# GewelsJI/MVLT

Measured on AMD Instinct MI355X. Metric: image-text pairs/sec/node, PVT-tiny MVLT pre-train step, higher is better.
Workload: dtype bf16

## Files before the change

mvlt_amd/_lib.py:

```python
import ctypes as C
import os

import torch

_HERE = os.path.dirname(os.path.abspath(__file__))
LIB_PATH = os.environ.get("MVLT_HIP_LIB") or os.path.join(_HERE, "libmvlt_hip.so")


class MVLTError(RuntimeError):
    pass


if not os.path.exists(LIB_PATH):
    raise ImportError(f"{LIB_PATH} is missing: build it with `python -m mvlt_amd.build` (hipcc, gfx950). "
                      "mvlt_amd has no CPU or eager fallback.")
lib = C.CDLL(LIB_PATH)

c_int, c_float, c_void_p, c_long = C.c_int, C.c_float, C.c_void_p, C.c_long


class RowMap(C.Structure):
    _fields_ = [(n, c_int) for n in ("mode", "rows_per_batch", "batch_stride", "offset",
                                     "r", "w_in", "tokens_in", "hw_out", "w_out", "c_seg", "h_in")]

# ... 140 lines not shown
    "mvlt_upsample_fwd": (_i, [_vp, _i, _i, _i, _i, _i, _i, _vp, _i, _i, _i, _vp]),
    "mvlt_upsample_bwd": (_i, [_vp, _i, _i, _i, _i, _i, _i, _i, _vp, _i, _i, _i, _i, _vp]),
    "mvlt_upsample_l1_fwd": (_i, [_vp, _i, _i, _i, _i, _i, _i, _vp, _vp, _vp]),
    "mvlt_upsample_l1_bwd": (_i, [_vp, _i, _i, _i, _i, _i, _i, _vp, _vp, _vp, _i, _i, _vp]),
}
EXPORTS = list(PROTOTYPES)
for _name, (_res, _args) in PROTOTYPES.items():
    _fn = getattr(lib, _name)
    _fn.restype, _fn.argtypes = _res, _args

ABI_VERSION = 8
if lib.mvlt_abi_version() != ABI_VERSION:
    raise ImportError(f"ABI mismatch: {LIB_PATH} is version {lib.mvlt_abi_version()}, the binding is version {ABI_VERSION} (stale build? run python -m mvlt_amd.build)")
for _name, _cls in STRUCTS:
    _n = lib.mvlt_sizeof(_name.encode())
    if _n != C.sizeof(_cls):
        raise ImportError(f"ABI mismatch for {_name}: library says {_n} bytes, binding has {C.sizeof(_cls)}")

EXT_PROTOTYPES = {
    "mvlt_ext_version": (_i, []),
    "mvlt_step_gate": (_i, [_vp, _i, _f, _f, _vp, _vp, _vp]),
    "mvlt_adamw_step_gated": (_i, [_vp, _vp, _vp, _vp, _vp, _l, _vp, _vp, _vp, _vp]),
}
for _name, (_res, _args) in EXT_PROTOTYPES.items():
    if not hasattr(lib, _name):
        raise ImportError(f"{LIB_PATH} does not export {_name} (include/mvlt_hip_ext.h): stale build? run python -m mvlt_amd.build")
    _fn = getattr(lib, _name)
    _fn.restype, _fn.argtypes = _res, _args

EXT_VERSION = 1
if lib.mvlt_ext_version() != EXT_VERSION:
    raise ImportError(f"extension mismatch: {LIB_PATH} is version {lib.mvlt_ext_version()}, the binding is version {EXT_VERSION} (stale build? run python -m mvlt_amd.build)")

DT = {torch.bfloat16: 0, torch.float32: 1}


def last_kernel():
    s = lib.mvlt_last_kernel().decode()
    s = s.replace("(anonymous namespace)::", "")
    if s.startswith("void "):
        s = s[5:]
    depth = 0
    for i, ch in enumerate(s):
        depth += ch == "<"
        depth -= ch == ">"
        if ch == "(" and depth == 0:
            return s[:i]
    return s


def check(rc, what):
    if rc != 0:
        raise MVLTError(f"{what} failed ({rc}): {lib.mvlt_last_error().decode()}")


_raw_stream, _cur_device = torch._C._cuda_getCurrentRawStream, torch._C._cuda_getDevice


def stream_ptr():
    return _raw_stream(_cur_device())


def ptr(t):
    if t is None:
        return None
    if not t.is_cuda:
# ... 15 lines not shown
```

mvlt_amd/build.py:

```python
import concurrent.futures
import os
import subprocess
import sys

HERE = os.path.dirname(os.path.abspath(__file__))
CSRC = os.path.join(HERE, "csrc")
OBJ = os.path.join(HERE, "csrc", "_obj")
LIB = os.path.join(HERE, "libmvlt_hip.so")
ARCH = "gfx950"
FLAGS = ["--offload-arch=" + ARCH, "-O3", "-std=c++17", "-fPIC", "-ffp-contract=fast", "-Wno-unused-result"]
EXTRA = {"mlp.hip": ["-fno-slp-vectorize"]}


def _sources():
    return sorted(f for f in os.listdir(CSRC) if f.endswith(".hip"))


def source_hash():
    import hashlib
    h = hashlib.sha256()
    files = sorted(os.path.join(CSRC, f) for f in os.listdir(CSRC) if f.endswith((".hip", ".h", ".inc")))
    files += [os.path.join(HERE, "..", "include", h) for h in ("mvlt_hip.h", "mvlt_hip_ext.h")]
    for f in files:
        h.update(os.path.basename(f).encode())
        h.update(open(f, "rb").read())
    return h.hexdigest()[:16]


def _deps_mtime():
    hdrs = [os.path.join(CSRC, f) for f in os.listdir(CSRC) if f.endswith((".h", ".inc"))]
    hdrs += [os.path.join(HERE, "..", "include", h) for h in ("mvlt_hip.h", "mvlt_hip_ext.h")]
    return max(os.path.getmtime(h) for h in hdrs)


def _compile(src, force, verbose):
    s = os.path.join(CSRC, src)
    o = os.path.join(OBJ, src[:-4] + ".o")
    if not force and os.path.exists(o) and os.path.getmtime(o) >= max(os.path.getmtime(s), _deps_mtime()):
        return o
    cmd = ["hipcc", *FLAGS, *EXTRA.get(src, []), "-c", s, "-o", o]
    if verbose:
        print(" ".join(cmd), flush=True)
    r = subprocess.run(cmd, capture_output=True, text=True)
    if r.returncode != 0:
        raise RuntimeError(f"hipcc failed for {src}:\n{r.stdout}\n{r.stderr}")
    return o


def build(force=False, verbose=False):
    os.makedirs(OBJ, exist_ok=True)
    srcs = _sources()
    with concurrent.futures.ThreadPoolExecutor(max_workers=min(6, len(srcs))) as ex:
        objs = list(ex.map(lambda s: _compile(s, force, verbose), srcs))
    if force or not os.path.exists(LIB) or any(os.path.getmtime(o) > os.path.getmtime(LIB) for o in objs):
        cmd = ["hipcc", "--offload-arch=" + ARCH, "-shared", "-fPIC", *objs, "-o", LIB]
        if verbose:
            print(" ".join(cmd), flush=True)
        r = subprocess.run(cmd, capture_output=True, text=True)
        if r.returncode != 0:
            raise RuntimeError(f"link failed:\n{r.stdout}\n{r.stderr}")
    return LIB


if __name__ == "__main__":
# ... 2 lines not shown
```

mvlt_amd/csrc/elementwise.hip:

```cpp
#include "common.h"
#include "../../include/mvlt_hip.h"
#include "../../include/mvlt_hip_ext.h"

namespace {

constexpr int NT = 256;

template <typename T, int HID>
__global__ __launch_bounds__(NT) void bert_embed_fwd_kernel(const long* ids, const float* word, const float* pos, const float* type0,
                                                            const float* gamma, const float* beta, const uint8_t* keep, float inv_keep,
                                                            T* y, float* mean_out, float* rstd_out, int rows, int Tlen, float eps) {
  constexpr int PER = HID / 64;
  const int lane = threadIdx.x & 63;
  const int row = blockIdx.x * (NT / 64) + (threadIdx.x >> 6);
  if (row >= rows) return;
  const long id = ids[row];
  const int t = row % Tlen;
  float v[PER];
  float s = 0.f;
#pragma unroll
  for (int i = 0; i < PER; ++i) {
    int c = lane + 64 * i;
    v[i] = word[id * HID + c] + type0[c] + pos[(long)t * HID + c];
    s += v[i];
  }
  const float mean = wave_sum(s) * (1.0f / HID);
  float q = 0.f;
#pragma unroll
  for (int i = 0; i < PER; ++i) { float d = v[i] - mean; q += d * d; }
  const float rstd = rsqrtf(wave_sum(q) * (1.0f / HID) + eps);
  if (lane == 0) { mean_out[row] = mean; rstd_out[row] = rstd; }
#pragma unroll
  for (int i = 0; i < PER; ++i) {
    int c = lane + 64 * i;
    float o = (v[i] - mean) * rstd * gamma[c] + beta[c];
// ... 261 lines not shown
    loss_sum[0] += L;
    count[0] += Cn;
  }
}

template <typename T, typename TO>
__global__ __launch_bounds__(NT) void ce_bwd_kernel(const T* logits, const long* labels, long ignore, const float* lse, const float* gscale,
                                                    const float* count, TO* dlogits, int rows, int V, int ld, int ldd) {
  const int row = blockIdx.x;
  const T* lr = logits + (long)row * ld;
  TO* dr = dlogits + (long)row * ldd;
  const long lab = labels[row];
  const float l = lse[row];
  const float sc = (lab == ignore) ? 0.f : gscale[0] / fmaxf(count[0], 1.0f);
  int c_first = 0;
  if constexpr (sizeof(T) == 4) {
    if ((ld & 3) == 0 && (ldd & 3) == 0 && (((uintptr_t)logits) & 15) == 0 && (((uintptr_t)dlogits) & 15) == 0) {
      const int V4 = V & ~3;
      for (int c = threadIdx.x * 4; c < V4; c += NT * 4) {
        const f32x4 x = *(const f32x4*)((const float*)lr + c);
        f32x4 g;
#pragma unroll
        for (int e = 0; e < 4; ++e) g[e] = (__expf(x[e] - l) - (c + e == lab ? 1.f : 0.f)) * sc;
        if constexpr (sizeof(TO) == 2) *(bf16x4*)((bf16*)dr + c) = bf16x4{(bf16)g[0], (bf16)g[1], (bf16)g[2], (bf16)g[3]};
        else *(f32x4*)((float*)dr + c) = g;
      }
      c_first = V4;
    }
  }
  for (int c = c_first + threadIdx.x; c < ldd; c += NT) {
    float g = 0.f;
    if (c < V) g = (__expf((float)lr[c] - l) - (c == lab ? 1.f : 0.f)) * sc;
    dr[c] = (TO)g;
  }
}

__global__ __launch_bounds__(NT) void smooth_l1_sum_kernel(const float* pred, const float* target, long n, float* loss_sum) {
  __shared__ float s_w[NT / 64];
  float acc = 0.f;
  const long stride = (long)gridDim.x * NT * 4;
  long i = ((long)blockIdx.x * NT + threadIdx.x) * 4;
  for (; i + 3 * stride < n; i += 4 * stride) {
    f32x4 a[4], b[4];
#pragma unroll
    for (int u = 0; u < 4; ++u) { a[u] = *(const f32x4*)(pred + i + u * stride); b[u] = *(const f32x4*)(target + i + u * stride); }
#pragma unroll
    for (int u = 0; u < 4; ++u)
#pragma unroll
      for (int e = 0; e < 4; ++e) {
        const float d = fabsf(a[u][e] - b[u][e]);
        acc += d < 1.0f ? 0.5f * d * d : d - 0.5f;
      }
  }
  for (; i < n; i += stride) {
    const f32x4 a = *(const f32x4*)(pred + i), b = *(const f32x4*)(target + i);
#pragma unroll
    for (int e = 0; e < 4; ++e) {
      const float d = fabsf(a[e] - b[e]);
      acc += d < 1.0f ? 0.5f * d * d : d - 0.5f;
    }
  }
  acc = wave_sum(acc);
  if ((threadIdx.x & 63) == 0) s_w[threadIdx.x >> 6] = acc;
  __syncthreads();
  if (threadIdx.x == 0) {
    float t = 0.f;
// ... 552 lines not shown

extern "C" int mvlt_smooth_l1_fwd(const float* pred, const float* target, long n, float* loss_sum, void* stream) {
  MVLT_REQUIRE(pred && target && loss_sum && n > 0 && n % 4 == 0 && (((uintptr_t)pred | (uintptr_t)target) & 15) == 0,
               "mvlt_smooth_l1_fwd: bad arguments (n multiple of 4, 16-byte aligned)");
  MVLT_LAUNCH(smooth_l1_sum_kernel, dim3(grid_for(n / 4, 2048)), dim3(NT), 0, (hipStream_t)stream, pred, target, n, loss_sum);
  return mvlt_check_launch("mvlt_smooth_l1_fwd");
}

extern "C" int mvlt_smooth_l1_bwd(const float* pred, const float* target, long n, const float* gscale, float* grad, void* stream) {
  MVLT_REQUIRE(pred && target && gscale && grad && n > 0 && n % 4 == 0 && (((uintptr_t)pred | (uintptr_t)target | (uintptr_t)grad) & 15) == 0,
               "mvlt_smooth_l1_bwd: bad arguments (n multiple of 4, 16-byte aligned)");
  MVLT_LAUNCH(smooth_l1_grad_kernel, dim3(grid_for(n / 4, 8192)), dim3(NT), 0, (hipStream_t)stream, pred, target, n, gscale, 1.0f / (float)n, grad);
  return mvlt_check_launch("mvlt_smooth_l1_bwd");
}

extern "C" int mvlt_adamw_step(float* p, const float* g, float* m, float* v, void* p_bf16, long n, const float* hp,
                               const uint8_t* decay_mask, const float* gscale_dev, void* stream) {
  MVLT_REQUIRE(p && g && m && v && hp && n >= 0 && n % 4 == 0, "mvlt_adamw_step: bad arguments (n must be a multiple of 4)");
  if (n == 0) return MVLT_OK;
  MVLT_LAUNCH((adamw_kernel<false>), dim3(grid_for(n / 4, 8192)), dim3(NT), 0, (hipStream_t)stream, p, g, m, v, (bf16*)p_bf16, n, hp, decay_mask, gscale_dev);
  return mvlt_check_launch("mvlt_adamw_step");
}

extern "C" int mvlt_ext_version(void) { return MVLT_EXT_VERSION; }

extern "C" int mvlt_adamw_step_gated(float* p, const float* g, float* m, float* v, void* p_bf16, long n, const float* hp,
                                     const uint8_t* decay_mask, const float* gate, void* stream) {
  MVLT_REQUIRE(p && g && m && v && hp && gate && n >= 0 && n % 4 == 0, "mvlt_adamw_step_gated: bad arguments (null pointer, or n is not a multiple of 4)");
  if (n == 0) return MVLT_OK;
  MVLT_LAUNCH((adamw_kernel<true>), dim3(grid_for(n / 4, 8192)), dim3(NT), 0, (hipStream_t)stream, p, g, m, v, (bf16*)p_bf16, n, hp, decay_mask, gate);
  return mvlt_check_launch("mvlt_adamw_step_gated");
}

extern "C" int mvlt_step_gate(const float* partials, int n_partials, float grad_scale, float max_norm, float* out, int* counters, void* stream) {
  MVLT_REQUIRE(partials && out && counters, "mvlt_step_gate: null pointer (partials, out and counters are required)");
  MVLT_REQUIRE(n_partials >= 1 && n_partials <= 1024, "mvlt_step_gate: n_partials must be in [1, 1024], got %d", n_partials);
  MVLT_LAUNCH(step_gate_kernel, dim3(1), dim3(NT), 0, (hipStream_t)stream, partials, n_partials, grad_scale, max_norm, out, counters);
  return mvlt_check_launch("mvlt_step_gate");
}

extern "C" int mvlt_grad_sumsq(const float* g, long n, const uint8_t* mask, float* partials, int n_partials, void* stream) {
  MVLT_REQUIRE(g && partials && n >= 0 && n % 4 == 0, "mvlt_grad_sumsq: bad arguments (n must be a multiple of 4)");
  MVLT_REQUIRE(n_partials >= 1 && n_partials <= 1024, "mvlt_grad_sumsq: n_partials must be in [1, 1024], got %d", n_partials);
  MVLT_REQUIRE(((uintptr_t)g & 15) == 0 && ((uintptr_t)mask & 3) == 0, "mvlt_grad_sumsq: g must be 16-byte aligned, mask 4-byte aligned");
  if (mask) MVLT_LAUNCH((grad_sumsq_kernel<true>), dim3(n_partials), dim3(NT), 0, (hipStream_t)stream, g, n, mask, partials);
  else MVLT_LAUNCH((grad_sumsq_kernel<false>), dim3(n_partials), dim3(NT), 0, (hipStream_t)stream, g, n, mask, partials);
  return mvlt_check_launch("mvlt_grad_sumsq");
}

extern "C" int mvlt_clip_coef(const float* partials, int n_partials, float grad_scale, float max_norm, float* out, void* stream) {
  MVLT_REQUIRE(partials && out && n_partials >= 1 && n_partials <= 1024, "mvlt_clip_coef: bad arguments (n_partials must be in [1, 1024])");
  MVLT_LAUNCH(clip_coef_kernel, dim3(1), dim3(NT), 0, (hipStream_t)stream, partials, n_partials, grad_scale, max_norm, out);
  return mvlt_check_launch("mvlt_clip_coef");
}

extern "C" int mvlt_scale_by_dev(float* x, long n, const float* factor_dev, void* stream) {
  MVLT_REQUIRE(x && factor_dev && n >= 0 && n % 4 == 0 && ((uintptr_t)x & 15) == 0, "mvlt_scale_by_dev: bad arguments (n must be a multiple of 4, x 16-byte aligned)");
  if (n == 0) return MVLT_OK;
  MVLT_LAUNCH(scale_by_dev_kernel, dim3(grid_for(n / 4, 8192)), dim3(NT), 0, (hipStream_t)stream, x, n, factor_dev);
  return mvlt_check_launch("mvlt_scale_by_dev");
}

extern "C" int mvlt_cast_bf16(const float* src, void* dst, long n, void* stream) {
  MVLT_REQUIRE(src && dst && n >= 0 && n % 4 == 0, "mvlt_cast_bf16: bad arguments (n must be a multiple of 4)");
  if (n == 0) return MVLT_OK;
  MVLT_LAUNCH(cast_f32_bf16_kernel, dim3(grid_for(n / 4, 8192)), dim3(NT), 0, (hipStream_t)stream, src, (bf16*)dst, n);
// ... 54 lines not shown
```

mvlt_amd/engine.py:

```python
import math

import torch
import torch.nn.functional as F

from ._lib import MVLTError
from .metrics import MetricLogger, SmoothedValue
from .params import pool_zeros

MLM_LOSS_WEIGHT, ITM_LOSS_WEIGHT, T2I_LOSS_WEIGHT = 1, 1, 10
USE_ORI_INPUT_IDS = False


def _core(model):
    return model.module if hasattr(model, "module") else model


class _SmoothL1Fn(torch.autograd.Function):

    @staticmethod
    def forward(ctx, pred, target):
        from . import ops
        pred, target = pred.contiguous(), target.contiguous()
        acc = pool_zeros((1,), torch.float32, pred.device)
        ops.smooth_l1_fwd(pred, target, acc)
# ... 152 lines not shown
        self.pin.copy_(vals, non_blocking=True)
        self.ev.record()

    def get(self):
        self.ev.synchronize()
        return self.pin.tolist()


def to_device_batch(samples, device):
    keys = ("image", "mlm_labels", "i2t_labels", "masked_images", "itm_labels", "sup_cls_labels", "sub_cls_labels")
    batch = {k: samples[k].to(device, non_blocking=True) for k in keys if k in samples}
    batch["input_ids"] = samples["ori_input_ids" if USE_ORI_INPUT_IDS else "input_ids"].to(device, non_blocking=True)
    if "mlm_positions" in samples:
        batch["mlm_positions"] = samples["mlm_positions"].to(device, non_blocking=True)
    if "mlm_count" in samples:
        batch["mlm_count"] = int(samples["mlm_count"])
    elif "mlm_positions" not in samples and not samples["mlm_labels"].is_cuda:
        batch["mlm_count"] = int((samples["mlm_labels"] != -1).sum())
    return batch


def train_one_epoch_vl(model, criterion, data_loader, optimizer, device, epoch, loss_scaler, max_norm=0,
                       model_ema=None, mixup_fn=None, set_training_mode=True, fp32=False, args=None):
    model.train(set_training_mode)
    core = _core(model)
    if fp32 and getattr(core, "compute_dtype", None) not in (None, torch.float32):
        core.set_compute_dtype(torch.float32)
    logger = MetricLogger(delimiter="  ")
    logger.add_meter("lr", SmoothedValue(window_size=1, fmt="{value:.6f}"))
    header = f"Epoch: [{epoch}]"
    loss_type = getattr(args, "loss_type", None) or core.loss_type
    t2i_on = loss_type.get("t2i", 0) == 1
    readback = _LossReadback()
    for idx, samples in enumerate(logger.log_every(data_loader, 10, header)):
        batch = to_device_batch(samples, device)
        total, parts = train_step(model, batch, idx, t2i_on)
        readback.post(total, parts)
        optimizer.zero_grad()
        is_second_order = hasattr(optimizer, "is_second_order") and optimizer.is_second_order
        loss_scaler(total, optimizer, clip_grad=max_norm, parameters=model.parameters(), create_graph=is_second_order)
        if model_ema is not None:
            model_ema.update(model)
        vals = readback.get()
        if not math.isfinite(vals[0]):
            print(f" [ Warning!!! ] Total Loss is {vals[0]} (loss_mlm={vals[1]} | loss_itm={vals[2]} | loss_sup_cls={vals[3]} | "
                  f"loss_sub_cls={vals[4]} | loss_t2i={vals[5]}), non-finite value"
                  + (" -- the step is guarded: non-finite gradients skip the optimizer step" if getattr(loss_scaler, "skip_nonfinite", False) else ""))
        logger.update(**dict(zip(LOSS_KEYS, vals)))
        logger.update(lr=optimizer.param_groups[0]["lr"])
    logger.synchronize_between_processes(device)
    print("Averaged stats:", logger)
    return {k: m.global_avg for k, m in logger.meters.items()}


train_one_epoch = train_one_epoch_vl


class BF16Scaler:
    state_dict_key = "amp_scaler"

    def __init__(self, skip_nonfinite=False):
        self._scaler = None
        self.skip_nonfinite = bool(skip_nonfinite)
        self.skipped_steps = 0
        self.last_grad_norm = None

    def __call__(self, loss, optimizer, clip_grad=None, parameters=None, create_graph=False):
        from .optim import FusedAdamW
        store = optimizer.model.store if isinstance(optimizer, FusedAdamW) else None
        self.last_grad_norm = None
        if store is not None:
            store.scale_in_optimizer = True
        try:
            loss.backward(create_graph=create_graph)
            if self.skip_nonfinite and store is not None:
                self.last_grad_norm = store.gate_grads(clip_grad or None)
            elif self.skip_nonfinite:
                assert parameters is not None
                parameters = list(parameters)
                norm = torch.nn.utils.clip_grad_norm_(parameters, clip_grad if clip_grad else float("inf"))
                if not math.isfinite(float(norm)):
                    self.skipped_steps += 1
                    return
            elif clip_grad and store is not None:
                self.last_grad_norm = store.clip_grad_norm(clip_grad)
            elif clip_grad:
                assert parameters is not None
                parameters = list(parameters)
                torch.nn.utils.clip_grad_norm_(parameters, clip_grad)
            optimizer.step()
        finally:
            if store is not None:
                store.scale_in_optimizer = False
                store.apply_pending_scale()

    def state_dict(self):
        return {}

    def load_state_dict(self, sd):
        pass
```

mvlt_amd/ops.py:

```python
import ctypes as C

import torch

from . import _lib as L
from ._lib import DT, check, patchmap, ptr, rowmap, stream_ptr

_ID = rowmap()


def gemm_nt(A, B, C_out, M, N, K, lda, ldb, ldc, *, a_map=None, c_map=None, bias=None, act=0, H=None,
            row_scale=None, rows_per_scale=0, R=None, col_sum=None, col_sumsq=None, col_copies=0, split_k=0, post_ln=None):
    assert A.dtype == B.dtype and A.dtype in DT and (C_out.dtype in DT or (C_out.dtype == torch.float16 and col_sum is not None))
    if bias is not None:
        assert bias.dtype == torch.float32
    if row_scale is not None:
        assert row_scale.dtype == torch.float32
    if R is not None:
        assert R.dtype == C_out.dtype or (R.dtype == torch.float32 and C_out.dtype == torch.bfloat16)
    if H is not None:
        assert H.dtype == C_out.dtype
    if col_sum is not None:
        assert col_sum.dtype == torch.float32 and col_sumsq is not None and col_sumsq.dtype == torch.float32
    a = L.GemmNTArgs(A=ptr(A), B=ptr(B), C=ptr(C_out), M=M, N=N, K=K, lda=lda, ldb=ldb, ldc=ldc,
                     dtype=DT[A.dtype], out_dtype=2 if C_out.dtype == torch.float16 else DT[C_out.dtype], a_map=a_map or _ID, c_map=c_map or _ID,
# ... 155 lines not shown


def masked_select(labels, idx, count, ignore_index=-1):
    assert labels.dtype == torch.int64 and idx.dtype == torch.int32 and count.dtype == torch.int32 and labels.is_contiguous()
    check(L.lib.mvlt_masked_select(ptr(labels), labels.numel(), ignore_index, ptr(idx), ptr(count), stream_ptr()), "mvlt_masked_select")


def gather_rows(src, idx, dst, rows, Cdim, ld_src, src_map=None):
    assert idx.dtype == torch.int32 and src.dtype == dst.dtype
    m = C.byref(src_map) if src_map is not None else None
    check(L.lib.mvlt_gather_rows(ptr(src), ptr(idx), ptr(dst), rows, Cdim, ld_src, m, DT[src.dtype], stream_ptr()), "mvlt_gather_rows")
    return dst


def scatter_rows(src, idx, dst, rows, Cdim, ld_dst, dst_map=None, accumulate=False):
    assert idx.dtype == torch.int32 and src.dtype == dst.dtype
    m = C.byref(dst_map) if dst_map is not None else None
    check(L.lib.mvlt_scatter_rows(ptr(src), ptr(idx), ptr(dst), rows, Cdim, ld_dst, m, 1 if accumulate else 0, DT[src.dtype], stream_ptr()),
          "mvlt_scatter_rows")
    return dst


def cross_entropy_fwd(logits, labels, lse, loss_sum, count, rows, V, ld, ignore_index=-1):
    assert labels.dtype == torch.int64
    check(L.lib.mvlt_cross_entropy_fwd(ptr(logits), ptr(labels), ignore_index, ptr(lse), ptr(loss_sum), ptr(count), rows, V, ld,
                                       DT[logits.dtype], stream_ptr()), "mvlt_cross_entropy_fwd")


def cross_entropy_bwd(logits, labels, lse, gscale, count, dlogits, rows, V, ld, ldd, ignore_index=-1):
    check(L.lib.mvlt_cross_entropy_bwd(ptr(logits), ptr(labels), ignore_index, ptr(lse), ptr(gscale), ptr(count), ptr(dlogits), rows, V, ld, ldd,
                                       DT[logits.dtype], DT[dlogits.dtype], stream_ptr()), "mvlt_cross_entropy_bwd")


ADAMW_FROZEN = 2


def adamw_step(p, g, m, v, p16, n, hp, decay_mask=None, *, gscale_dev=None):
    assert decay_mask is None or decay_mask.dtype == torch.uint8
    if gscale_dev is not None:
        assert gscale_dev.dtype == torch.float32
    check(L.lib.mvlt_adamw_step(ptr(p), ptr(g), ptr(m), ptr(v), ptr(p16), n, ptr(hp), ptr(decay_mask), ptr(gscale_dev), stream_ptr()), "mvlt_adamw_step")


def grad_sumsq(g, n, mask, partials):
    assert g.dtype == torch.float32 and partials.dtype == torch.float32 and g.is_contiguous() and partials.is_contiguous()
    assert g.numel() >= n and (mask is None or (mask.dtype == torch.uint8 and mask.is_cuda and mask.is_contiguous() and mask.numel() >= n))
    check(L.lib.mvlt_grad_sumsq(ptr(g), n, ptr(mask), ptr(partials), partials.numel(), stream_ptr()), "mvlt_grad_sumsq")


def clip_coef(partials, grad_scale, max_norm, out):
    assert partials.dtype == torch.float32 and out.dtype == torch.float32 and out.numel() >= 2 and out.is_contiguous() and partials.is_contiguous()
    check(L.lib.mvlt_clip_coef(ptr(partials), partials.numel(), float(grad_scale), float(max_norm), ptr(out), stream_ptr()), "mvlt_clip_coef")


def step_gate(partials, grad_scale, max_norm, out, counters):
    assert partials.dtype == torch.float32 and out.dtype == torch.float32 and out.numel() >= 4 and out.is_contiguous() and partials.is_contiguous()
    assert counters.dtype == torch.int32 and counters.numel() >= 2 and counters.is_contiguous()
    check(L.lib.mvlt_step_gate(ptr(partials), partials.numel(), float(grad_scale), float(max_norm), ptr(out), ptr(counters), stream_ptr()), "mvlt_step_gate")


def adamw_step_gated(p, g, m, v, p16, n, hp, decay_mask, gate):
    assert decay_mask is None or decay_mask.dtype == torch.uint8
    assert gate.dtype == torch.float32 and gate.numel() >= 4 and gate.is_contiguous()
    check(L.lib.mvlt_adamw_step_gated(ptr(p), ptr(g), ptr(m), ptr(v), ptr(p16), n, ptr(hp), ptr(decay_mask), ptr(gate), stream_ptr()), "mvlt_adamw_step_gated")


# ... 221 lines not shown
```

mvlt_amd/params.py:

```python
import math
import weakref
from collections import OrderedDict

import torch
import torch.nn as nn

from . import ops

_TN_SCRATCH_MIB = 256
ALIGN = 8


class Holder(nn.Module):

    def __init__(self, **shapes):
        super().__init__()
        for name, shape in shapes.items():
            self.register_parameter(name, nn.Parameter(torch.zeros(*shape)))


def affine(n):
    return Holder(weight=(n,), bias=(n,))


# ... 62 lines not shown
        self.used += nbytes
        return t


def pool_zeros(shape, dtype, device):
    return ZeroPool.of(torch.device(device) if not isinstance(device, torch.device) else device).take(tuple(shape) if not isinstance(shape, int) else (shape,), dtype)


class FlatStore:

    def __init__(self, module, compute_dtype):
        self.module = module
        self.compute_dtype = compute_dtype
        self.device = None
        self.P = self.G = self.C = None
        self._views = {}
        self.offsets = OrderedDict()
        self.params = OrderedDict()
        self.total = 0
        self._cast_version = -1
        self.refresh_count = 0
        self._c_fresh_version = None
        self.extra = {}
        self._finalize_queued = False
        self.force_dirty = True
        self.fn_params = []
        self.on_backward_done = None
        self.on_range_ready = None
        self.on_pass_aborted = None
        self._ranges_done = []
        self.all_zeroed_this_pass = False
        self.touched_this_pass = set()
        self.scale_in_optimizer = False
        self.pending_grad_scale = 1.0
        self.pending_clip = None
        self._clip = None
        self.pending_gate = None
        self._gate = None
        self.grad_works = []

    def _index(self):
        self.offsets.clear()
        self.params.clear()
        off = 0
        seen = set()
        for name, p in self.module.named_parameters():
            if id(p) in seen:
                continue
            seen.add(id(p))
            n = p.numel()
            self.offsets[name] = (off, n, tuple(p.shape))
            self.params[name] = p
            off += (n + ALIGN - 1) // ALIGN * ALIGN
        self.total = off
        self.fn_params = list(self.params.items())

    def is_current(self):
        if self.P is None:
            return False
        for name in (next(iter(self.params)), next(reversed(self.params))):
            off, n, _ = self.offsets[name]
            if self.params[name].data_ptr() != self.P.data_ptr() + 4 * off:
                return False
        return True

    def materialize(self, device):
# ... 377 lines not shown
```

mvlt_amd/schedule.py:

```python
import torch
import torch.nn.functional as F

from . import ops
from ._lib import patchmap, rowmap
from .params import ZeroPool, pool_zeros
from .pvlt import BERT_DROP, EPS_BERT, EPS_BLOCK, EPS_DEFAULT, VOCAB, VOCAB_LD


def _empty(shape, dtype, dev):
    return torch.empty(shape, dtype=dtype, device=dev)


def conv_wgrad(S, name, dz, xin, M, cout, K, ld_dz, ld_in, bmap, taps, cin, colsum=None):
    ops.gemm_tn(dz, xin, S.grad_taps(name, cout, taps, cin), M, cout, K, ld_dz, ld_in, K, b_map=bmap, colsum=colsum, partials=S.tn_partials(), defer_fold=True)


def _step_rng(model):
    model._rng_calls = getattr(model, "_rng_calls", 0) + 1
    return torch.initial_seed(), model._rng_calls


def check_input_size(model, Himg, Wimg):
    unit = model.patch_size * 8
    assert Himg % unit == 0 and Wimg % unit == 0, \
# ... 815 lines not shown
    @staticmethod
    def backward(ctx, dlogits):
        model, HW, x4, e, sv_e, t, sv_t, a_map, sink = ctx.pack
        S, dt, dev = model.store, model.compute_dtype, x4.device
        S.queue_finalize()
        B, N, C = x4.shape
        T = N - HW
        R = B * T
        dl = torch.zeros(R, VOCAB_LD, device=dev, dtype=dt)
        dl[:, :VOCAB] = dlogits.reshape(R, VOCAB).to(dt)
        u = ctx.unit
        dx4, ret = (sink or _GradSink(S)).take(x4.shape, dt, dev) if u.dgrad else (None, None)
        _mlm_decoder_bwd(model, dl, t, sv_t, e, sv_e, x4, a_map, R, C, dx4, accumulate=True, unit=u)
        ctx.pack = ctx.unit = None
        return ret, None, None, None


def _mlm_decoder_bwd(model, dl, t, sv_t, e, sv_e, A, a_map, R, lda, dA, c_map=None, accumulate=False, unit=_EVERY):
    S, dt, dev = model.store, model.compute_dtype, dl.device
    Hd = model.hidden
    wname = WORD_TABLE
    if unit.launches["table"]:
        ops.gemm_tn(dl, t, S.grad(wname), R, VOCAB, Hd, VOCAB_LD, Hd, Hd, colsum=S.grad("mlm_head.bias"),
                    overwrite=dt == torch.bfloat16 and S.all_zeroed_this_pass and wname not in S.touched_this_pass)
        S.touched_this_pass.add(wname)
    elif unit.launches["bias"]:
        db = _empty((1, VOCAB_LD), torch.float32, dev)
        ops.batch_sum(dl, db, R, 1, VOCAB_LD, 1, VOCAB_LD)
        S.grad("mlm_head.bias").add_(db[0, :VOCAB])
    wT = S.extra[wname + "::T"]
    if dt == torch.bfloat16:
        dtr32 = pool_zeros((R, Hd), torch.float32, dev)
        ops.gemm_nt(dl, wT, dtr32, R, Hd, VOCAB_LD, VOCAB_LD, VOCAB_LD, Hd, split_k=4)
        dtr = dtr32.to(dt)
    else:
        dtr = _empty((R, Hd), dt, dev)
        ops.gemm_nt(dl, wT, dtr, R, Hd, VOCAB_LD, VOCAB_LD, VOCAB_LD, Hd)
    de = _mlm_transform_bwd(model, dtr, sv_t, e, R, unit)
    _embed_ln_bwd(model, "mlm_head_embed", de, sv_e, A, a_map, R, lda, dA, c_map if c_map is not None else a_map, accumulate, unit)
    S.announce_prefix("mlm_head_embed.", "mlm_head.")


class _MLMFusedFn(torch.autograd.Function):

    @staticmethod
    def forward(ctx, x4, model, HW, positions, labels_sel, sink):
        S, dt, dev = model.store, model.compute_dtype, x4.device
        B, N, C = x4.shape
        T = N - HW
        R = positions.numel()
        rows = _empty((R, C), dt, dev)
        tmap = rowmap(T, N, HW)
        ops.gather_rows(x4, positions, rows, R, C, C, src_map=tmap)
        e, sv_e = _embed_ln_fwd(model, "mlm_head_embed", rows, None, R, C)
        t, sv_t = _mlm_transform_fwd(model, e, R)
        logits = _empty((R, VOCAB_LD), torch.float32, dev)
        ops.gemm_nt(t, S.comp("text_embeddings.word_embeddings.weight"), logits, R, VOCAB, model.hidden, model.hidden, model.hidden, VOCAB_LD,
                    bias=S.master("mlm_head.bias"))
        lse = _empty((R,), torch.float32, dev)
        acc = pool_zeros((2,), torch.float32, dev)
        ops.cross_entropy_fwd(logits, labels_sel, lse, acc[0:1], acc[1:2], R, VOCAB, VOCAB_LD)
        ctx.pack = (model, HW, x4.shape, rows, e, sv_e, t, sv_t, logits, lse, acc, positions, labels_sel, tmap, sink)
        ctx.unit = _unit(getattr(model, "_plan", None), "mlm_head")
        return acc[0] / acc[1]

    @staticmethod
    def backward(ctx, gloss):
        model, HW, xshape, rows, e, sv_e, t, sv_t, logits, lse, acc, positions, labels_sel, tmap, sink = ctx.pack
        S, dt, dev = model.store, model.compute_dtype, rows.device
        S.queue_finalize()
        B, N, C = xshape
        R = positions.numel()
        dl = _empty((R, VOCAB_LD), dt, dev)
        gs = gloss.reshape(1).float().contiguous()
        ops.cross_entropy_bwd(logits, labels_sel, lse, gs, acc[1:2], dl, R, VOCAB, VOCAB_LD, VOCAB_LD)
        u = ctx.unit
        drows = _empty((R, C), dt, dev) if u.dgrad else None
        _mlm_decoder_bwd(model, dl, t, sv_t, e, sv_e, rows, None, R, C, drows, c_map=None, unit=u)
        ret = None
        if u.dgrad:
            dx4, ret = (sink or _GradSink(S)).take(xshape, dt, dev)
            ops.scatter_rows(drows, positions, dx4, R, C, C, dst_map=tmap, accumulate=True)
        ctx.pack = ctx.unit = None
        return ret, None, None, None, None, None


class _HostCount:
    _pins = {}

    def __init__(self, cnt):
        key = (cnt.device.index, cnt.numel())
        pin = self._pins.get(key)
        if pin is None:
            pin = self._pins[key] = torch.empty(cnt.numel(), dtype=cnt.dtype).pin_memory()
        self.pin = pin
        pin.copy_(cnt, non_blocking=True)
        self.ev = torch.cuda.Event()
        self.ev.record()

    def get(self):
        self.ev.synchronize()
        return int(self.pin[0])


def run_forward(model, images, ids, mlm_labels=None, mlm_positions=None, mlm_count=None, t2i_target=None):
    S = model.store
    dev = images.device
    grad_on = _begin_pass(model, dev)
# ... 77 lines not shown
```

Measured before the change: 13520.

## Fuse MLM cross-entropy forward and backward into one kernel during forward

Adds a fused HIP kernel that computes the log-sum-exp and writes the logit gradient in a single pass over each row, launched in the forward pass with a precomputed upstream loss weight. This saves re-reading the fp32 logits in backward and one kernel launch, and lets the logits buffer be freed early. The backward path only rescales the gradient if the promised upstream weight was not honoured. It also swaps a torch dtype conversion for the library's bf16 cast op. The risk is that gradients are wrong if the actual upstream scale differs from the announced weight, and the extra plumbing across engine, store and schedule makes that easy to get out of sync.

```diff
diff --git a/include/mvlt_hip_ext2.h b/include/mvlt_hip_ext2.h
--- /dev/null
+++ b/include/mvlt_hip_ext2.h
@@ -0,0 +1,19 @@
+#ifndef MVLT_HIP_EXT2_H
+#define MVLT_HIP_EXT2_H
+#include <stdint.h>
+#ifdef __cplusplus
+extern "C" {
+#endif
+
+#define MVLT_EXT2_VERSION 1
+int mvlt_ext2_version(void);
+
+#define MVLT_CE_FUSED_MAX_V 32768
+#define MVLT_CE_FUSED_MAX_GRID 2048
+int mvlt_cross_entropy_fwd_bwd(const void* logits, const long* labels, long ignore_index, float* lse, float* loss_sum, float* count,
+                               const float* gscale , void* dlogits, int rows, int V, int ld, int ldd, int dtype, int out_dtype, void* stream);
+
+#ifdef __cplusplus
+}
+#endif
+#endif
diff --git a/mvlt_amd/_lib.py b/mvlt_amd/_lib.py
--- a/mvlt_amd/_lib.py
+++ b/mvlt_amd/_lib.py
@@ -196,6 +196,20 @@
 if lib.mvlt_ext_version() != EXT_VERSION:
     raise ImportError(f"extension mismatch: {LIB_PATH} is version {lib.mvlt_ext_version()}, the binding is version {EXT_VERSION} (stale build? run python -m mvlt_amd.build)")
 
+EXT2_PROTOTYPES = {
+    "mvlt_ext2_version": (_i, []),
+    "mvlt_cross_entropy_fwd_bwd": (_i, [_vp, _vp, _l, _vp, _vp, _vp, _vp, _vp, _i, _i, _i, _i, _i, _i, _vp]),
+}
+for _name, (_res, _args) in EXT2_PROTOTYPES.items():
+    if not hasattr(lib, _name):
+        raise ImportError(f"{LIB_PATH} does not export {_name} (include/mvlt_hip_ext2.h): stale build? run python -m mvlt_amd.build)")
+    _fn = getattr(lib, _name)
+    _fn.restype, _fn.argtypes = _res, _args
+
+EXT2_VERSION = 1
+if lib.mvlt_ext2_version() != EXT2_VERSION:
+    raise ImportError(f"extension mismatch: {LIB_PATH} is version {lib.mvlt_ext2_version()} of mvlt_hip_ext2.h, the binding is version {EXT2_VERSION} (stale build? run python -m mvlt_amd.build)")
+
 DT = {torch.bfloat16: 0, torch.float32: 1}
 
 
diff --git a/mvlt_amd/build.py b/mvlt_amd/build.py
--- a/mvlt_amd/build.py
+++ b/mvlt_amd/build.py
@@ -10,6 +10,7 @@
 ARCH = "gfx950"
 FLAGS = ["--offload-arch=" + ARCH, "-O3", "-std=c++17", "-fPIC", "-ffp-contract=fast", "-Wno-unused-result"]
 EXTRA = {"mlp.hip": ["-fno-slp-vectorize"]}
+ABI_HEADERS = ("mvlt_hip.h", "mvlt_hip_ext.h", "mvlt_hip_ext2.h")
 
 
 def _sources():
@@ -20,7 +21,7 @@
     import hashlib
     h = hashlib.sha256()
     files = sorted(os.path.join(CSRC, f) for f in os.listdir(CSRC) if f.endswith((".hip", ".h", ".inc")))
-    files += [os.path.join(HERE, "..", "include", h) for h in ("mvlt_hip.h", "mvlt_hip_ext.h")]
+    files += [os.path.join(HERE, "..", "include", h) for h in ABI_HEADERS]
     for f in files:
         h.update(os.path.basename(f).encode())
         h.update(open(f, "rb").read())
@@ -29,7 +30,7 @@
 
 def _deps_mtime():
     hdrs = [os.path.join(CSRC, f) for f in os.listdir(CSRC) if f.endswith((".h", ".inc"))]
-    hdrs += [os.path.join(HERE, "..", "include", h) for h in ("mvlt_hip.h", "mvlt_hip_ext.h")]
+    hdrs += [os.path.join(HERE, "..", "include", h) for h in ABI_HEADERS]
     return max(os.path.getmtime(h) for h in hdrs)
 
 
diff --git a/mvlt_amd/csrc/elementwise.hip b/mvlt_amd/csrc/elementwise.hip
--- a/mvlt_amd/csrc/elementwise.hip
+++ b/mvlt_amd/csrc/elementwise.hip
@@ -1,6 +1,7 @@
 #include "common.h"
 #include "../../include/mvlt_hip.h"
 #include "../../include/mvlt_hip_ext.h"
+#include "../../include/mvlt_hip_ext2.h"
 
 namespace {
 
@@ -328,6 +329,103 @@
     float g = 0.f;
     if (c < V) g = (__expf((float)lr[c] - l) - (c == lab ? 1.f : 0.f)) * sc;
     dr[c] = (TO)g;
+  }
+}
+
+constexpr int CE_NT = 1024;
+template <typename T, typename TO, int NCH>
+__global__ __launch_bounds__(CE_NT) void ce_fwd_bwd_kernel(const T* logits, const long* labels, long ignore, float* lse, const float* gscale,
+                                                           TO* dlogits, int rows, int V, int ld, int ldd) {
+  constexpr int PC = 16 / sizeof(T), NW = CE_NT / 64;
+  __shared__ float s_m[NW], s_s[NW];
+  __shared__ int s_c[NW];
+  const int tid = threadIdx.x, lane = tid & 63, wave = tid >> 6;
+  float x[NCH * PC];
+  auto load_row = [&](int r) {
+    const T* lr = logits + (long)r * ld;
+    u32x4 raw[NCH];
+#pragma unroll
+    for (int u = 0; u < NCH; ++u) {
+      const int c = (u * CE_NT + tid) * PC;
+      raw[u] = *(const u32x4*)(lr + (c < V ? c : 0));
+    }
+#pragma unroll
+    for (int u = 0; u < NCH; ++u) {
+      const int left = V - (u * CE_NT + tid) * PC;
+#pragma unroll
+      for (int e = 0; e < PC; ++e) {
+        float v;
+        if constexpr (sizeof(T) == 4) v = __builtin_bit_cast(f32x4, raw[u])[e];
+        else v = (float)__builtin_bit_cast(bf16x8, raw[u])[e];
+        x[u * PC + e] = e < left ? v : -INFINITY;
+      }
+    }
+  };
+  int row = blockIdx.x;
+  load_row(row);
+  int cnt = 0;
+#pragma unroll 1
+  for (int r = tid; r < rows; r += CE_NT) cnt += labels[r] != ignore ? 1 : 0;
+#pragma unroll
+  for (int o = 32; o > 0; o >>= 1) cnt += __shfl_xor(cnt, o);
+  if (lane == 0) s_c[wave] = cnt;
+  __syncthreads();
+  int labelled = 0;
+#pragma unroll
+  for (int w = 0; w < NW; ++w) labelled += s_c[w];
+  const float per_row = gscale[0] / fmaxf((float)labelled, 1.0f);
+  for (;;) {
+    const long lab = labels[row];
+    float m = x[0];
+#pragma unroll
+    for (int i = 1; i < NCH * PC; ++i) m = fmaxf(m, x[i]);
+    m = wave_max(m);
+    if (lane == 0) s_m[wave] = m;
+    __syncthreads();
+    float M = s_m[0];
+#pragma unroll
+    for (int w = 1; w < NW; ++w) M = fmaxf(M, s_m[w]);
+    float s = 0.f;
+#pragma unroll
+    for (int i = 0; i < NCH * PC; i += 4) {
+#pragma unroll
+      for (int e = 0; e < 4; ++e) x[i + e] = __expf(x[i + e] - M);
+      s += (x[i] + x[i + 1]) + (x[i + 2] + x[i + 3]);
+    }
+    s = wave_sum(s);
+    if (lane == 0) s_s[wave] = s;
+    __syncthreads();
+    float S = s_s[0];
+#pragma unroll
+    for (int w = 1; w < NW; ++w) S += s_s[w];
+    if (tid == 0) lse[row] = M + logf(S);
+    const bool live = lab != ignore;
+    const int labi = (int)lab;
+    const float inv = 1.0f / S;
+    const float sc = live ? per_row : 0.f;
+    TO* dr = dlogits + (long)row * ldd;
+#pragma unroll
+    for (int u = 0; u < NCH; ++u) {
+      const int c = (u * CE_NT + tid) * PC;
+      if (c < ldd) {
+        float g[PC];
+        const int hot = labi - c;
+#pragma unroll
+        for (int e = 0; e < PC; ++e) g[e] = live ? (x[u * PC + e] * inv - (e == hot ? 1.f : 0.f)) * sc : 0.f;
+        if constexpr (sizeof(TO) == 2) {
+          if constexpr (PC == 4) *(bf16x4*)((bf16*)dr + c) = bf16x4{(bf16)g[0], (bf16)g[1], (bf16)g[2], (bf16)g[3]};
+          else *(bf16x8*)((bf16*)dr + c) = bf16x8{(bf16)g[0], (bf16)g[1], (bf16)g[2], (bf16)g[3], (bf16)g[4], (bf16)g[5], (bf16)g[6], (bf16)g[7]};
+        } else {
+#pragma unroll
+          for (int q = 0; q < PC; q += 4) *(f32x4*)((float*)dr + c + q) = f32x4{g[q], g[q + 1], g[q + 2], g[q + 3]};
+        }
+      }
+    }
+#pragma unroll 1
+    for (int c = NCH * CE_NT * PC + tid; c < ldd; c += CE_NT) dr[c] = (TO)0.f;
+    row += gridDim.x;
+    if (row >= rows) break;
+    load_row(row);
   }
 }
 
@@ -946,6 +1044,44 @@
   return mvlt_check_launch("mvlt_adamw_step_gated");
 }
 
+extern "C" int mvlt_ext2_version(void) { return MVLT_EXT2_VERSION; }
+
+template <typename T, typename TO>
+static void ce_fwd_bwd_launch(int nch, dim3 grid, hipStream_t s, const void* logits, const long* labels, long ignore, float* lse, const float* gscale,
+                              void* dlogits, int rows, int V, int ld, int ldd) {
+#define MVLT_CE_CASE(N) MVLT_LAUNCH((ce_fwd_bwd_kernel<T, TO, N>), grid, dim3(CE_NT), 0, s, (const T*)logits, labels, ignore, lse, gscale, (TO*)dlogits, rows, V, ld, ldd)
+  if (nch <= 1) MVLT_CE_CASE(1);
+  else if (nch <= 2) MVLT_CE_CASE(2);
+  else if (nch <= 4) MVLT_CE_CASE(4);
+  else if constexpr (sizeof(T) == 4) MVLT_CE_CASE(8);
+#undef MVLT_CE_CASE
+}
+
+extern "C" int mvlt_cross_entropy_fwd_bwd(const void* logits, const long* labels, long ignore_index, float* lse, float* loss_sum, float* count,
+                                          const float* gscale, void* dlogits, int rows, int V, int ld, int ldd, int dtype, int out_dtype, void* stream) {
+  MVLT_REQUIRE(logits && labels && lse && loss_sum && count && gscale && dlogits, "mvlt_cross_entropy_fwd_bwd: null pointer");
+  MVLT_REQUIRE((dtype == 0 || dtype == 1) && (out_dtype == 0 || out_dtype == 1), "mvlt_cross_entropy_fwd_bwd: dtype / out_dtype must be 0 (bf16) or 1 (fp32)");
+  MVLT_REQUIRE(V > 0 && ld >= V && ldd >= V, "mvlt_cross_entropy_fwd_bwd: need V > 0, ld >= V and ldd >= V (V %d, ld %d, ldd %d)", V, ld, ldd);
+  const int esz = dtype == 0 ? 2 : 4, osz = out_dtype == 0 ? 2 : 4, pc = 16 / esz;
+  MVLT_REQUIRE(((long)ld * esz) % 16 == 0 && ((long)ldd * osz) % 16 == 0 && ldd % pc == 0 && (((uintptr_t)logits | (uintptr_t)dlogits) & 15) == 0,
+               "mvlt_cross_entropy_fwd_bwd: logits / dlogits and their row pitches must be 16-byte aligned (ld %d, ldd %d; ldd a multiple of %d)", ld, ldd, pc);
+  if (rows <= 0) return MVLT_OK;
+  if (V > MVLT_CE_FUSED_MAX_V) {
+    const int rc = mvlt_cross_entropy_fwd(logits, labels, ignore_index, lse, loss_sum, count, rows, V, ld, dtype, stream);
+    return rc != MVLT_OK ? rc : mvlt_cross_entropy_bwd(logits, labels, ignore_index, lse, gscale, count, dlogits, rows, V, ld, ldd, dtype, out_dtype, stream);
+  }
+  hipStream_t s = (hipStream_t)stream;
+  const dim3 grid(rows < MVLT_CE_FUSED_MAX_GRID ? rows : MVLT_CE_FUSED_MAX_GRID);
+  const int nch = (V + CE_NT * pc - 1) / (CE_NT * pc);
+  if (dtype == 1 && out_dtype == 0) ce_fwd_bwd_launch<float, bf16>(nch, grid, s, logits, labels, ignore_index, lse, gscale, dlogits, rows, V, ld, ldd);
+  else if (dtype == 1) ce_fwd_bwd_launch<float, float>(nch, grid, s, logits, labels, ignore_index, lse, gscale, dlogits, rows, V, ld, ldd);
+  else if (out_dtype == 0) ce_fwd_bwd_launch<bf16, bf16>(nch, grid, s, logits, labels, ignore_index, lse, gscale, dlogits, rows, V, ld, ldd);
+  else ce_fwd_bwd_launch<bf16, float>(nch, grid, s, logits, labels, ignore_index, lse, gscale, dlogits, rows, V, ld, ldd);
+  if (dtype == 0) MVLT_LAUNCH((ce_loss_finish_kernel<bf16>), dim3(1), dim3(1024), 0, s, (const bf16*)logits, labels, ignore_index, (const float*)lse, loss_sum, count, rows, ld);
+  else MVLT_LAUNCH((ce_loss_finish_kernel<float>), dim3(1), dim3(1024), 0, s, (const float*)logits, labels, ignore_index, (const float*)lse, loss_sum, count, rows, ld);
+  return mvlt_check_launch("mvlt_cross_entropy_fwd_bwd");
+}
+
 extern "C" int mvlt_step_gate(const float* partials, int n_partials, float grad_scale, float max_norm, float* out, int* counters, void* stream) {
   MVLT_REQUIRE(partials && out && counters, "mvlt_step_gate: null pointer (partials, out and counters are required)");
   MVLT_REQUIRE(n_partials >= 1 && n_partials <= 1024, "mvlt_step_gate: n_partials must be in [1, 1024], got %d", n_partials);
diff --git a/mvlt_amd/engine.py b/mvlt_amd/engine.py
--- a/mvlt_amd/engine.py
+++ b/mvlt_amd/engine.py
@@ -208,9 +208,14 @@
     loss_type = getattr(args, "loss_type", None) or core.loss_type
     t2i_on = loss_type.get("t2i", 0) == 1
     readback = _LossReadback()
+    announce = isinstance(loss_scaler, BF16Scaler) and hasattr(core, "store")
     for idx, samples in enumerate(logger.log_every(data_loader, 10, header)):
         batch = to_device_batch(samples, device)
-        total, parts = train_step(model, batch, idx, t2i_on)
+        core._mlm_upstream = float(MLM_LOSS_WEIGHT) if announce else None
+        try:
+            total, parts = train_step(model, batch, idx, t2i_on)
+        finally:
+            core._mlm_upstream = None
         readback.post(total, parts)
         optimizer.zero_grad()
         is_second_order = hasattr(optimizer, "is_second_order") and optimizer.is_second_order
@@ -247,8 +252,13 @@
         self.last_grad_norm = None
         if store is not None:
             store.scale_in_optimizer = True
+            store.upstream_promised = True
         try:
-            loss.backward(create_graph=create_graph)
+            try:
+                loss.backward(create_graph=create_graph)
+            finally:
+                if store is not None:
+                    store.upstream_promised = False
             if self.skip_nonfinite and store is not None:
                 self.last_grad_norm = store.gate_grads(clip_grad or None)
             elif self.skip_nonfinite:
diff --git a/mvlt_amd/ops.py b/mvlt_amd/ops.py
--- a/mvlt_amd/ops.py
+++ b/mvlt_amd/ops.py
@@ -211,6 +211,15 @@
                                        DT[logits.dtype], DT[dlogits.dtype], stream_ptr()), "mvlt_cross_entropy_bwd")
 
 
+CE_FUSED_MAX_V, CE_FUSED_MAX_GRID = 32768, 2048
+
+
+def cross_entropy_fwd_bwd(logits, labels, lse, loss_sum, count, gscale, dlogits, rows, V, ld, ldd, ignore_index=-1):
+    assert labels.dtype == torch.int64 and gscale.dtype == torch.float32 and lse.dtype == loss_sum.dtype == count.dtype == torch.float32
+    check(L.lib.mvlt_cross_entropy_fwd_bwd(ptr(logits), ptr(labels), ignore_index, ptr(lse), ptr(loss_sum), ptr(count), ptr(gscale), ptr(dlogits),
+                                           rows, V, ld, ldd, DT[logits.dtype], DT[dlogits.dtype], stream_ptr()), "mvlt_cross_entropy_fwd_bwd")
+
+
 ADAMW_FROZEN = 2
 
 
diff --git a/mvlt_amd/params.py b/mvlt_amd/params.py
--- a/mvlt_amd/params.py
+++ b/mvlt_amd/params.py
@@ -118,6 +118,7 @@
         self.all_zeroed_this_pass = False
         self.touched_this_pass = set()
         self.scale_in_optimizer = False
+        self.upstream_promised = False
         self.pending_grad_scale = 1.0
         self.pending_clip = None
         self._clip = None
diff --git a/mvlt_amd/schedule.py b/mvlt_amd/schedule.py
--- a/mvlt_amd/schedule.py
+++ b/mvlt_amd/schedule.py
@@ -871,13 +871,21 @@
     if dt == torch.bfloat16:
         dtr32 = pool_zeros((R, Hd), torch.float32, dev)
         ops.gemm_nt(dl, wT, dtr32, R, Hd, VOCAB_LD, VOCAB_LD, VOCAB_LD, Hd, split_k=4)
-        dtr = dtr32.to(dt)
+        dtr = _empty((R, Hd), dt, dev)
+        ops.cast_bf16(dtr32, dtr, R * Hd)
     else:
         dtr = _empty((R, Hd), dt, dev)
         ops.gemm_nt(dl, wT, dtr, R, Hd, VOCAB_LD, VOCAB_LD, VOCAB_LD, Hd)
     de = _mlm_transform_bwd(model, dtr, sv_t, e, R, unit)
     _embed_ln_bwd(model, "mlm_head_embed", de, sv_e, A, a_map, R, lda, dA, c_map if c_map is not None else a_map, accumulate, unit)
     S.announce_prefix("mlm_head_embed.", "mlm_head.")
+
+
+def _upstream_dev(model, value, dev):
+    hit = getattr(model, "_mlm_upstream_dev", None)
+    if hit is None or hit[0] != (value, dev):
+        hit = model._mlm_upstream_dev = ((value, dev), torch.full((1,), value, device=dev, dtype=torch.float32))
+    return hit[1]
 
 
 class _MLMFusedFn(torch.autograd.Function):
@@ -898,21 +906,32 @@
                     bias=S.master("mlm_head.bias"))
         lse = _empty((R,), torch.float32, dev)
         acc = pool_zeros((2,), torch.float32, dev)
-        ops.cross_entropy_fwd(logits, labels_sel, lse, acc[0:1], acc[1:2], R, VOCAB, VOCAB_LD)
-        ctx.pack = (model, HW, x4.shape, rows, e, sv_e, t, sv_t, logits, lse, acc, positions, labels_sel, tmap, sink)
+        up = getattr(model, "_mlm_upstream", None)
+        dl = None
+        if up is not None and dt == torch.bfloat16 and getattr(model, "_plan", None) is not None:
+            gs = _upstream_dev(model, up, dev)
+            dl = _empty((R, VOCAB_LD), dt, dev)
+            ops.cross_entropy_fwd_bwd(logits, labels_sel, lse, acc[0:1], acc[1:2], gs, dl, R, VOCAB, VOCAB_LD, VOCAB_LD)
+            logits = lse = None
+        else:
+            ops.cross_entropy_fwd(logits, labels_sel, lse, acc[0:1], acc[1:2], R, VOCAB, VOCAB_LD)
+        ctx.pack = (model, HW, x4.shape, rows, e, sv_e, t, sv_t, logits, lse, acc, positions, labels_sel, tmap, sink, dl, up)
         ctx.unit = _unit(getattr(model, "_plan", None), "mlm_head")
         return acc[0] / acc[1]
 
     @staticmethod
     def backward(ctx, gloss):
-        model, HW, xshape, rows, e, sv_e, t, sv_t, logits, lse, acc, positions, labels_sel, tmap, sink = ctx.pack
+        model, HW, xshape, rows, e, sv_e, t, sv_t, logits, lse, acc, positions, labels_sel, tmap, sink, dl, up = ctx.pack
         S, dt, dev = model.store, model.compute_dtype, rows.device
         S.queue_finalize()
         B, N, C = xshape
         R = positions.numel()
-        dl = _empty((R, VOCAB_LD), dt, dev)
-        gs = gloss.reshape(1).float().contiguous()
-        ops.cross_entropy_bwd(logits, labels_sel, lse, gs, acc[1:2], dl, R, VOCAB, VOCAB_LD, VOCAB_LD)
+        if dl is None:
+            dl = _empty((R, VOCAB_LD), dt, dev)
+            gs = gloss.reshape(1).float().contiguous()
+            ops.cross_entropy_bwd(logits, labels_sel, lse, gs, acc[1:2], dl, R, VOCAB, VOCAB_LD, VOCAB_LD)
+        elif not getattr(S, "upstream_promised", False):
+            dl.mul_((gloss.reshape(1).float() / up).to(dt))
         u = ctx.unit
         drows = _empty((R, C), dt, dev) if u.dgrad else None
         _mlm_decoder_bwd(model, dl, t, sv_t, e, sv_e, rows, None, R, C, drows, c_map=None, unit=u)
```

Measured after the change: 13530, median of 2. No clear change (+0.1%).
